# kalenforn/clip-based-cross-modal-hash

Hardware: AMD Instinct MI355X
Metric: Hamming query x gallery pairs/sec (fused mAP@all pass, DCMHT COCO-shaped 64-bit) (higher is better)
Workload: dtype u32; 1 GPU; configs[1] DCMHT COCO 64-bit retrieval: Q=5000 queries x R=117218 gallery items per GPU (x1 GPUs, contiguous shards), K=64 bits, C=80 classes, mAP@all; Q=5000, R_per_gpu=117218, K=64, C=80, parallelism=gallery-shard x1, query_blocks=1

## Files before the change

clip-based-cross-modal-hash_amd/csrc/xmh_scan.hip:

```cpp
#include "xmh_common.h"
#include <atomic>
#include <math.h>
#include <mutex>
#include <string.h>
#include <vector>
#include "xmh_scan_bits.h"
#include "xmh_scan_mfma.h"
#include "xmh_scan_kernels.h"

#include <stdlib.h>
#include <type_traits>

namespace {

constexpr int kSlotBudget64 = 9 * 1024;
constexpr int kSlotBudget32 = 5 * 1024;
constexpr int slots_for(int W, bool tern, int counter_bytes) {
    const int nbmax = (tern ? 64 : 32) * W + 1;
    const int budget = counter_bytes == 8 ? kSlotBudget64 : kSlotBudget32;
    const int cap = W > 8 ? 64 : 8;
    int S = 2;
    while (S < cap && nbmax * (64 / S) * counter_bytes > budget) S *= 2;
    return S;
}
inline int instance_words(int W) { return W <= 1 ? 1 : (W <= 2 ? 2 : (W <= 4 ? 4 : (W <= 8 ? 8 : (W <= 16 ? 16 : (W <= 32 ? 32 : 64))))); }
constexpr bool pair_cache_shape(int W, bool tern) { return !tern && (W == 1 || W == 2 || W == 4 || W == 8); }
// ... 247 lines not shown
    int W = 0, LW = 0;
    bool tern = false, cache = false;
    int S = 0, NW = 1;
    int nml = 0;
    int eb = 0; bool half = false;
    bool p32 = false, masked = false;
    unsigned gate = 0;
    bool stand_in = false;
};
struct ScanRoute {
    Launch p1;
    size_t cache_bytes = 0;
    int rank_bits = 0;
    Launch p2[3];
    int n2 = 0;
};

ScanRoute scan_route(const xmh_scan_plan& p, const ScanCall& c, Mode mode, const Overrides& ov, hipStream_t st) {
    ScanRoute r;
    const int K = c.K, C = c.C; const bool tern = c.tern; const int64_t R = c.R;
    const Family fam = pass1_family(K, tern, ov);
    const int W = ov.describe ? instance_words((K + 31) / 32) : (K + 31) / 32, LW = (C + 31) / 32;
    const bool lane_ok = ov.describe || (!ov.masked && lane_order_ok(st));
    r.cache_bytes = cache_for_workspace(p, K, tern, fam, c.ws_bytes);
    const bool cache = r.cache_bytes != 0;
    const bool mfma = fam != Family::kValu && LW <= 4 && lane_ok;
    Launch& h = r.p1;
    h.W = W; h.LW = LW; h.tern = tern; h.cache = cache; h.nml = LW <= 2 ? 1 : 2;
    if (!mfma) {
        h.cache = cache && pair_cache_shape(W, tern);
        h.S = h.cache ? cache_slots(W) : slots_for(W, tern, 4);
// ... 19 lines not shown
    const unsigned size_gate = sharded && (apc || apr2) ? kBySize : 0u;
    r.rank_bits = byte128 && apc ? 0 : rank_bits;
    auto add = [&](Kern kern, unsigned gate) -> Launch& { Launch& l = r.p2[r.n2++]; l.kern = kern; l.gate = gate; return l; };
    if (apc) {
        Launch& l = add(Kern::kApC, size_gate | (byte128 ? kByWrap : 0u));
        l.eb = 8; l.half = byte128; l.S = byte128 ? 8 : 4;
    }
    if (apr2) {
        Launch& l = add(Kern::kApR2, size_gate);
        l.W = W; l.LW = LW; l.nml = h.nml; l.NW = kAp2Waves; l.S = kAp2Groups;
    }
    if (apc16) {
        Launch& l = add(Kern::kApC, kByWidth);
        l.eb = 16; l.S = 8;
    }
    if ((apc || apr2) && !size_gate && !byte128) return r;
    Launch s;
    s.kern = Kern::kApS; s.W = tb ? 8 : W; s.LW = LW; s.tern = tern && !tb; s.masked = masked;
    s.cache = cache && !byte128 && !masked && pair_cache_shape(s.W, s.tern);
    s.stand_in = byte128 && apc;
    s.gate = size_gate | (s.stand_in ? kByWrap : 0u) | (r.rank_bits ? kByWidth : 0u);
    for (const bool p32 : {true, false}) {
        if (p32 ? r.rank_bits == 0 : apc16) continue;
        s.p32 = p32;
        s.S = s.cache ? cache_slots(s.W) : slots_for(s.W, s.tern, p32 ? 4 : 8);
        s.NW = s.S == 64 ? waves_for(s.W, s.tern) : 1;
        r.p2[r.n2++] = s;
    }
    return r;
}

// ... 80 lines not shown
    hipLaunchKernelGGL(kern, dim3(g.grid), dim3(g.block), g.lds, st, args...);
    return XMH_OK;
}

struct ScanCtx {
    const ScanCall& c;
    hipStream_t st;
    xmh_scan_plan p;
    ScanRoute r;
    WsLayout L;
    ScanArgs a;
    uint32_t kcap = 0xffffffffu;
    bool capped = false;
    template <typename T> T* at(size_t off) const { return reinterpret_cast<T*>(static_cast<char*>(c.ws) + off); }
    uint32_t* chunk_hist() const { return at<uint32_t>(L.chunk_hist); }
    const uint2* below() const { return at<uint2>(L.below); }
    uint2* tot() const { return at<uint2>(L.tot); }
    uint2* dpre() const { return at<uint2>(L.dpre); }
    uint32_t* cap_ws() const { return at<uint32_t>(L.cap); }
    float* ap_part() const { return at<float>(L.ap_part); }
    ScanArgs args(const Geom& g, bool cached) const { ScanArgs as = a; as.nqt = g.nqt; as.nrun = g.nrun; as.pair_cache = cached ? pair_cache() : nullptr; return as; }
    uint32_t* gate(int word = 0) const { return at<uint32_t>(L.gate) + word; }
    const uint32_t* gate_if(const Launch& l, unsigned g, int word) const { return (l.gate & g) ? gate(word) : nullptr; }
    uint4* pair_cache() const { return r.cache_bytes ? at<uint4>(L.pair_cache) : nullptr; }
};

int plan_call(const char* who, ScanCtx& x, const Overrides& ov) {
    if (const int rc = make_plan(x.c.Q, x.c.R, x.c.K, x.c.tern, &x.p, ov)) return rc;
    return check_common(who, x.c, x.p);
}
// ... 41 lines not shown
    hipLaunchKernelGGL(k_scan_touch, dim3(xmh::scan_grid_blocks(kTouchPerChunk, (int)p.nchunk)), dim3(256), 0, x.st, x.c.rbits, x.c.rlab, x.c.R, h.W, h.LW,
                       p.chunk, (int)p.nchunk, x.at<uint32_t>(x.L.tick), (int)((x.L.gate + 256 - x.L.tick) / 4));
    XMH_LAUNCH_CHECK("xmh_hamming_hist control words");
    const MfmaArgs a = r2_args(x.c, h, p, g.nqt);
    xmh::ProfScope prof("scan_hist", x.st);
    auto go = [&](auto kern, int NW, int NQ, bool cached, auto... wrap_word) { return start("xmh_hamming_hist", h, g, x.st, kern, NQ, NW, cached, a, chunk_hist, cache, wrap_word...); };
    if (h.kern == Kern::kHistR2w) {
        uint32_t* ovf = x.gate(kGateWrapped);
        return h.nml == 1 ? (h.cache ? go(k_scan_hist_r2w<1, 4, 2, true>, 4, 2, true, ovf) : go(k_scan_hist_r2w<1, 4, 2, false>, 4, 2, false, ovf))
                          : (h.cache ? go(k_scan_hist_r2w<2, 4, 2, true>, 4, 2, true, ovf) : go(k_scan_hist_r2w<2, 4, 2, false>, 4, 2, false, ovf));
    }
    return h.nml == 1 ? (h.cache ? go(k_scan_hist_r2<1, 4, 4, true>, 4, 4, true) : go(k_scan_hist_r2<1, 4, 4, false>, 4, 4, false))
                      : (h.cache ? go(k_scan_hist_r2<2, 4, 4, true>, 4, 4, true) : go(k_scan_hist_r2<2, 4, 4, false>, 4, 4, false));
}

int hamming_hist_impl(const ScanCall& c, uint32_t* hist_all, uint32_t* hist_rel, xmh_stream_t stream, const Overrides& ov) {
    ScanCtx x{c, xmh::as_stream(stream)};
    if (const int rc = plan_call("xmh_hamming_hist", x, ov)) return rc;
    route_call(x, Mode::kUnsharded, ov);
    const xmh_scan_plan& p = x.p;
    const Kern kern = x.r.p1.kern;
    if (kern == Kern::kHistS || kern == Kern::kHistB) XMH_HIP(hipMemsetAsync(x.at<char>(x.L.tick), 0, x.L.gate + 256 - x.L.tick, x.st));
    if (const int rc = kern == Kern::kHistS ? valu_hist(x) : mfma_hist(x)) return rc;
    XMH_LAUNCH_CHECK("xmh_hamming_hist");
    hipLaunchKernelGGL(k_scan_below, dim3((unsigned)p.nqtile, (unsigned)xmh::ceil_div(p.nbuckets, 4)), dim3(256), 0, x.st, x.chunk_hist(), (int)p.qpad,
                       (int)p.nbuckets, (int)p.nchunk, kern != Kern::kHistS ? kRelHi16 : 0u, x.at<uint2>(x.L.below), x.tot(), x.at<uint32_t>(x.L.tick), (int)c.Q, x.dpre(),
                       x.cap_ws(), x.gate(), hist_all, hist_rel);
    XMH_LAUNCH_CHECK("xmh_hamming_hist below");
    return XMH_OK;
}

}

extern "C" int xmh_scan_plan_make(int64_t Q, int64_t R, int K, int ternary, xmh_scan_plan* plan_host) {
    if (!plan_host) return xmh::fail(XMH_EINVAL, "xmh_scan_plan_make: null plan");
    return make_plan(Q, R, K, ternary, plan_host);
}

extern "C" size_t xmh_scan_pair_cache_bytes(int64_t Q, int64_t R, int K, int ternary) {
    xmh_scan_plan p;
    if (make_plan(Q, R, K, ternary, &p)) return 0;
    return pair_cache_bytes(p, K, ternary != 0, pass1_family(K, ternary != 0, {}));
}
// ... 19 lines not shown
    const ScanCall c{nullptr, nullptr, nullptr, nullptr, nullptr, nullptr, Q, R, K, C, nullptr, (size_t)p.ws_bytes, ternary != 0};
    const ScanRoute r = scan_route(p, c, Mode::kUnsharded, ov, nullptr);
    char p1[160], p2[200] = "", one[120];
    if (const int rc = describe_launch(r.p1, p1, sizeof(p1))) return rc;
    for (const bool p32 : {true, false})
        for (int i = 0; i < r.n2; ++i) {
            if (r.p2[i].stand_in || r.p2[i].p32 != p32) continue;
            if (const int rc = describe_launch(r.p2[i], one, sizeof(one))) return rc;
            const size_t at = strlen(p2);
            snprintf(p2 + at, sizeof(p2) - at, "%s%s", at ? "|" : "", one);
        }
    if ((size_t)snprintf(out, out_bytes, "pass1=%s;pass2=%s", p1, p2) >= out_bytes) return xmh::fail(XMH_EINVAL, "xmh_scan_describe: buffer too small");
    return XMH_OK;
}

extern "C" int xmh_hamming_hist(const uint32_t* qbits, const uint32_t* qzero, const uint32_t* qlab,
                                const uint32_t* rbits, const uint32_t* rzero, const uint32_t* rlab, int64_t Q, int64_t R,
                                int K, int C, void* ws, size_t ws_bytes, uint32_t* hist_all, uint32_t* hist_rel,
                                xmh_stream_t stream) {
    XMH_RANGE("xmh_hamming_hist (pass 1)");
    const ScanCall c{qbits, qzero, qlab, rbits, rzero, rlab, Q, R, K, C, ws, ws_bytes, qzero != nullptr};
    return hamming_hist_impl(c, hist_all, hist_rel, stream, {});
}

namespace {
int ap_offsets(const ScanCtx& x, const Pass2& o) {
    const xmh_scan_plan& p = x.p;
    if (o.mode == Mode::kUnsharded) return XMH_OK;
    if (o.mode == Mode::kAllToAll)
        hipLaunchKernelGGL(k_shard_scatter_offsets, dim3((unsigned)xmh::ceil_div(p.qpad, 256), (unsigned)p.nbuckets + 1), dim3(256), 0, x.st,
                           reinterpret_cast<const uint2*>(o.hist_g), (int)p.nbuckets, (int)(p.qpad / o.world), (int)x.c.Q, (int)p.qpad, o.k, x.dpre(), x.cap_ws(),
                           o.cap, x.gate(2));
    else if (o.mode == Mode::kTotals)
        hipLaunchKernelGGL(k_shard_offsets_dpre, dim3((unsigned)p.nqtile), dim3(256), 0, x.st, reinterpret_cast<const uint2*>(o.hist_g), o.world, o.rank,
                           (int)x.c.Q, (int)p.qpad, (int)p.nbuckets, o.k, x.dpre(), x.cap_ws(), o.cap, x.gate(2));
    else
        hipLaunchKernelGGL(k_scan_dpre, dim3((unsigned)p.nqtile), dim3(256), 0, x.st, (const uint2*)x.tot(), (int)x.c.Q, (int)p.qpad, (int)p.nbuckets, o.base_all,
                           o.base_rel, o.nrel_total, o.k, x.dpre(), x.cap_ws(), o.cap, (uint32_t*)nullptr, (uint32_t*)nullptr, (uint32_t*)nullptr, x.gate(2));
    XMH_LAUNCH_CHECK(o.mode == Mode::kAllToAll ? "xmh_hamming_map_sharded_offsets scatter" : (o.mode == Mode::kTotals ? "xmh_hamming_map_sharded offsets" : "xmh_hamming_ap dpre"));
    return XMH_OK;
}

int ap_launch_c(const ScanCtx& x, const Launch& l) {
    const Geom g = launch_geom(l, x.p, x.c.Q);
    const ScanArgs as = x.args(g, true);
    xmh::ProfScope prof("scan_ap", x.st);
    auto go = [&](auto kc, int S) {
        return start("xmh_hamming_ap", l, g, x.st, kc, S, 1, l.cache, as, x.below(), (const uint2*)x.dpre(), (const uint32_t*)x.cap_ws(), x.ap_part(),
                     x.gate_if(l, kBySize, 2), x.kcap, x.gate_if(l, kByWrap, kGateWrapped), x.gate_if(l, kByWidth, 0), l.gate & kByWidth ? x.r.rank_bits : 0);
    };
    if (l.eb == 16) return x.capped ? go(k_scan_ap_c<true, 16>, 8) : go(k_scan_ap_c<false, 16>, 8);
    if (l.half) return x.capped ? go(k_scan_ap_c<true, 8, true>, 8) : go(k_scan_ap_c<false, 8, true>, 8);
    return x.capped ? go(k_scan_ap_c<true, 8>, 4) : go(k_scan_ap_c<false, 8>, 4);
}

int ap_launch_r2(const ScanCtx& x, const Launch& l) {
    const Geom g = launch_geom(l, x.p, x.c.Q);
    const MfmaArgs ma = r2_args(x.c, l, x.p, g.nrun);
    xmh::ProfScope prof("scan_ap", x.st);
    auto go = [&](auto kern) {
        return start("xmh_hamming_ap", l, g, x.st, kern, kAp2Groups, kAp2Waves, l.cache, ma, x.below(), (const uint2*)x.dpre(), (const uint32_t*)x.cap_ws(), x.ap_part(),
                     x.gate_if(l, kBySize, 2), x.kcap);
    };
    return l.nml == 1 ? (x.capped ? go(k_scan_ap_r2<1, kAp2Waves, kAp2Groups, true>) : go(k_scan_ap_r2<1, kAp2Waves, kAp2Groups, false>))
// ... 91 lines not shown
    }
    if (nbad)
        return xmh::fail(XMH_EVERIFY_CODE, "xmh_scan_verify: %lld of %lld queries differ between the lane-order kernels and the masked re-derivation "
                         "(first: query %lld, AP sum %.9g vs %.9g, divisor %d vs %d)", (long long)nbad, (long long)Q, (long long)bad, a1[(size_t)bad], a0[(size_t)bad],
                         c1[(size_t)bad], c0[(size_t)bad]);
    return XMH_OK;
}

int hamming_ap_impl(const ScanCall& c, const Pass2& o, xmh_stream_t stream, const Overrides& ov) {
    ScanCtx x{c, xmh::as_stream(stream)};
    if (const int rc = plan_call("xmh_hamming_ap", x, ov)) return rc;
    if (!o.ap_sum || !o.cap) return xmh::fail(XMH_EINVAL, "xmh_hamming_ap: null output");
    const int ext = (o.base_all != nullptr) + (o.base_rel != nullptr) + (o.nrel_total != nullptr);
    if (ext != 0 && ext != 3) return xmh::fail(XMH_EINVAL, "xmh_hamming_ap: base_all, base_rel and nrel_total go together");
    route_call(x, o.mode, ov);
    x.kcap = o.k > 0 && o.k < (int64_t)0xffffffffll ? (uint32_t)o.k : 0xffffffffu;
    x.capped = o.k > 0;
    if (const int rc = ap_offsets(x, o)) return rc;
    for (int i = 0; i < x.r.n2; ++i) {
        const Launch& l = x.r.p2[i];
        if (const int rc = l.kern == Kern::kApC ? ap_launch_c(x, l) : (l.kern == Kern::kApR2 ? ap_launch_r2(x, l) : ap_launch_s(x, l))) return rc;
        XMH_LAUNCH_CHECK("xmh_hamming_ap");
    }
    if (const int rc = ap_reduce(x, o)) return rc;
    if (g_verify.load(std::memory_order_relaxed) && !ov.masked && o.mode == Mode::kUnsharded) return verify_against_masked(c, o, stream);
    return XMH_OK;
}

bool selfcheck_eval(const ScanCall& c, int force, std::vector<uint32_t>& hist, std::vector<double>& ap, std::vector<int32_t>& cap) {
    Overrides ov;
    ov.mfma = force;
    const int64_t Q = c.Q;
// ... 197 lines not shown
```

clip-based-cross-modal-hash_amd/csrc/xmh_scan_kernels.h:

```cpp
#pragma once
#include "xmh_scan_mfma.h"

namespace {
template <int W, int LW, bool TERN>
struct QueryRegs {
    uint32_t b[W];
    uint32_t z[TERN ? W : 1];
    uint32_t l[LW];
    __device__ __forceinline__ void load(const ScanArgs& a, int q) {
        const bool ok = q < a.Q;
#pragma unroll
        for (int w = 0; w < W; ++w) b[w] = ok ? a.qbits[(int64_t)q * W + w] : 0u;
        if (TERN) {
#pragma unroll
            for (int w = 0; w < W; ++w) z[w] = ok ? a.qzero[(int64_t)q * W + w] : 0xffffffffu;
        }
#pragma unroll
        for (int w = 0; w < LW; ++w) l[w] = ok ? a.qlab[(int64_t)q * LW + w] : 0u;
    }
};

template <int W, int LW, bool TERN>
struct Rec {
    uint32_t b[W];
// ... 12 lines not shown
        int live_n = 0, diff_n = 0;
#pragma unroll
        for (int w = 0; w < W; ++w) {
            const uint32_t live = ~(qr.z[w] | r.z[w]);
            live_n += __popc(live);
            diff_n += __popc((qr.b[w] ^ r.b[w]) & live);
        }
        d = K - live_n + 2 * diff_n;
    }
    uint32_t hit = qr.l[0] & r.l[0];
#pragma unroll
    for (int w = 1; w < LW; ++w) asm("v_and_or_b32 %0, %1, %2, %0" : "+v"(hit) : "v"(qr.l[w]), "v"(r.l[w]));
    asm("v_min_u32 %0, %1, 1" : "=v"(hit01) : "v"(hit));
}

constexpr uint32_t kRelHi16 = 0xffffffffu;
constexpr int kGateWrapped = 3;
__global__ __launch_bounds__(256) void k_scan_below(const uint32_t* __restrict__ chunk_hist, int qpad, int nb, int nchunk, uint32_t rel_scale,
                                                    uint2* __restrict__ below, uint2* __restrict__ tot, uint32_t* __restrict__ tickets, int Q,
                                                    uint2* __restrict__ dpre, uint32_t* __restrict__ nrel_ws, uint32_t* __restrict__ nrel_max,
                                                    uint32_t* __restrict__ hist_all, uint32_t* __restrict__ hist_rel) {
    __shared__ uint2 part[4][64];
    __shared__ int last;
    const int lane = threadIdx.x & 63, wq = threadIdx.x >> 6;
    const int d = blockIdx.y * 4 + wq;
    const int q = blockIdx.x * 64 + lane;
    const bool hi16 = rel_scale == kRelHi16;
    if (d < nb) {
        uint32_t ra = 0, rr = 0;
        int c = 0;
        for (; c + 4 <= nchunk; c += 4) {
            uint32_t h[4];
#pragma unroll
            for (int j = 0; j < 4; ++j) h[j] = chunk_hist[((int64_t)(c + j) * nb + d) * qpad + q];
#pragma unroll
            for (int j = 0; j < 4; ++j) {
                below[((int64_t)(c + j) * nb + d) * qpad + q] = make_uint2(ra, rr);
                const uint32_t rel = hi16 ? h[j] & 0xffffu : (rel_scale ? h[j] / rel_scale : h[j] >> 16);
                ra += hi16 ? h[j] >> 16 : (rel_scale ? h[j] - rel * rel_scale : h[j] & 0xffffu);
                rr += rel;
            }
        }
        for (; c < nchunk; ++c) {
// ... 878 lines not shown
```

clip-based-cross-modal-hash_amd/csrc/xmh_scan_mfma.h:

```cpp
#pragma once
#include "xmh_common.h"
#include "xmh_scan_map.h"
#include <type_traits>
#include <utility>

namespace {

constexpr int kMaxChunk = 32768;
constexpr uint32_t kF23 = 0x4B000000u;
constexpr int64_t kFloatBitsMaxItems = (1ll << 23) - 3;
constexpr int kMinChunk = 256;

struct ScanArgs {
    const uint32_t* qbits;
    const uint32_t* qzero;
    const uint32_t* qlab;
    const uint32_t* rbits;
    const uint32_t* rzero;
    const uint32_t* rlab;
    int Q, R, K;
    int chunk, nchunk, nqt, qpad, nb;
    uint4* pair_cache;
    int nrun;
};

__device__ __forceinline__ bool map_block(const ScanArgs& a, int& chunk_id, int& qtile) {
// ... 602 lines not shown
        uint32_t* __restrict__ out = chunk_hist + ((int64_t)chunk_id * a.nb) * a.qpad + (t16 + h) * 16;
        for (int e = lane; e < ncell; e += 64) out[(int64_t)(e >> 4) * a.qpad + (e & 15)] = lds[r2_cell(wave, h, e >> 4, e & 15)];
    }
    if (CACHE && dmax >= 65536u) *ovf = 1u;
}
#undef XMH_W_FUSED
#undef XMH_W_MFMA_F4
#undef XMH_W_MFMA
#undef XMH_W_MIN
#undef XMH_W_ADD

template <bool CAPPED, int EB, bool HALF = false>
__global__ __launch_bounds__(64) void k_scan_ap_c(ScanArgs a, const uint2* __restrict__ below, const uint2* __restrict__ dpre,
                                                  const uint32_t* __restrict__ cap_ws, float* __restrict__ ap_part,
                                                  const uint32_t* __restrict__ items_total, uint32_t kcap, const uint32_t* __restrict__ skip_if = nullptr,
                                                  const uint32_t* __restrict__ nrel_max = nullptr, int rank_bits = 0) {
    static_assert(!HALF || EB == 8, "the 8 x 8 geometry on one-byte entries");
    constexpr int QW = HALF ? 8 : 128 / EB, LOG_QW = QW == 16 ? 4 : 3, S = 64 / QW, EPW = HALF ? 2 : 32 / EB;
    extern __shared__ __attribute__((aligned(16))) uint32_t lds[];
    int chunk_id, qtile;
    if (!map_block(a, chunk_id, qtile)) return;
    if (items_total && (int64_t)*items_total > kFloatBitsMaxItems) return;
    if (skip_if && *skip_if != 0u) return;
    if (nrel_max && rank_bits > 0 && (uint64_t)(*nrel_max) + 2 < (1ull << (32 - rank_bits))) return;
    const int lane = threadIdx.x & 63;
    const int ql = lane & (QW - 1), slot = lane >> LOG_QW;
    const int q0 = qtile * QW, q = q0 + ql;
    const int ncell = a.nb * QW;
    unsigned long long* cnt = reinterpret_cast<unsigned long long*>(lds);
    {
        const uint2* __restrict__ pb = below + ((int64_t)chunk_id * a.nb) * a.qpad + q0;
        const uint2* __restrict__ pd = dpre + q0;
        auto pack = [](uint2 x, uint2 y) {
            return (unsigned long long)(kF23 + x.x + y.x + 1u) | ((unsigned long long)(kF23 + (0x7fffffu - (x.y + y.y + 1u))) << 32);
        };
        int e = lane;
        for (; e + 7 * 64 < ncell; e += 8 * 64) {
            uint2 x[8], y[8];
#pragma unroll
            for (int j = 0; j < 8; ++j) {
                const int ee = e + j * 64;
                const int64_t at = (int64_t)(ee >> LOG_QW) * a.qpad + (ee & (QW - 1));
                x[j] = pb[at];
                y[j] = pd[at];
            }
#pragma unroll
            for (int j = 0; j < 8; ++j) cnt[e + j * 64] = pack(x[j], y[j]);
        }
        for (; e < ncell; e += 64) {
            const int64_t at = (int64_t)(e >> LOG_QW) * a.qpad + (e & (QW - 1));
            cnt[e] = pack(pb[at], pd[at]);
        }
    }
    const uint32_t cntbase = (uint32_t)(uintptr_t)(__attribute__((address_space(3))) uint32_t*)lds + ql * 8;
    const float capf = CAPPED ? (float)min(cap_ws[q], kcap) : 0.0f;
    const int64_t lo = (int64_t)chunk_id * a.chunk;
    const int64_t hi = (lo + a.chunk < a.R) ? lo + a.chunk : a.R;
    float acc = 0.0f;
    auto credit = [&](unsigned long long old, uint32_t m) {
        const float rank = __uint_as_float((uint32_t)old) - 8388608.0f;
        const float ord = 16777215.0f - __uint_as_float((uint32_t)(old >> 32));
        if (CAPPED) m = ord <= capf ? m : 0u;
#ifdef XMH_ABL_AP_NORCP
        acc = fmaf(ord, __uint_as_float(__float_as_uint(rank) & m), acc);
#else
        acc = fmaf(ord, __uint_as_float(__float_as_uint(__builtin_amdgcn_rcpf(rank)) & m), acc);
#endif
    };
// ... 448 lines not shown
```

clip-based-cross-modal-hash_amd/xmh/_lib.py:

```python
from __future__ import annotations

import ctypes as C
import os

_HERE = os.path.dirname(os.path.abspath(__file__))
LIB_PATH = os.environ.get("XMH_LIB", os.path.join(_HERE, "libxmh.so"))

if not os.path.exists(LIB_PATH):
    raise ImportError(
        "libxmh.so not found at %s -- build it first (python -c 'import __graft_entry__ as g; g.build()' "
        "or make -C clip-based-cross-modal-hash_amd). There is no CPU fallback." % LIB_PATH)

import torch

lib = C.CDLL(LIB_PATH)

vp, i64, i32, sz = C.c_void_p, C.c_int64, C.c_int, C.c_size_t


class ScanPlan(C.Structure):
    _fields_ = [("chunk", i64), ("nchunk", i64), ("nqtile", i64), ("qpad", i64), ("nbuckets", i64), ("ws_bytes", sz)]


class Linear(C.Structure):
# ... 120 lines not shown
    "xmh_range_push": (i32, [C.c_char_p]),
    "xmh_range_pop": (i32, []),
    "xmh_scan_verify": (i32, [i32]),
    "xmh_prof_read": (i32, [C.c_char_p, C.POINTER(C.c_double), C.POINTER(i64)]),
    "xmh_pack_sign": (i32, [vp, i64, i32, vp, vp, vp, vp, vp]),
    "xmh_pack_pair_argmax": (i32, [vp, i64, i32, vp, vp, vp]),
    "xmh_unpack_pm1": (i32, [vp, vp, i64, i32, vp, vp]),
    "xmh_pack_labels": (i32, [vp, i32, i64, i32, vp, vp]),
    "xmh_hamming_dist": (i32, [vp, vp, vp, vp, i64, i64, i32, vp, vp, vp]),
    "xmh_label_sim": (i32, [vp, vp, i64, i64, i32, vp, vp]),
    "xmh_scan_plan_make": (i32, [i64, i64, i32, i32, C.POINTER(ScanPlan)]),
    "xmh_scan_pair_cache_bytes": (sz, [i64, i64, i32, i32]),
    "xmh_scan_pair_cache_offset": (sz, [i64, i64, i32, i32]),
    "xmh_scan_ws_bytes_nocache": (sz, [i64, i64, i32, i32]),
    "xmh_scan_describe": (i32, [i64, i64, i32, i32, i32, C.c_char_p, sz]),
    "xmh_hamming_hist": (i32, [vp, vp, vp, vp, vp, vp, i64, i64, i32, i32, vp, sz, vp, vp, vp]),
    "xmh_hamming_ap": (i32, [vp, vp, vp, vp, vp, vp, i64, i64, i32, i32, vp, sz, vp, vp, vp, i64, vp, vp, vp]),
    "xmh_hamming_map": (i32, [vp, vp, vp, vp, vp, vp, i64, i64, i32, i32, vp, sz, i64, vp, vp, vp, vp]),
    "xmh_scan_totals_offset": (sz, [i64, i64, i32, i32, C.POINTER(C.c_size_t)]),
    "xmh_hamming_map_sharded": (i32, [vp, vp, vp, vp, vp, vp, i64, i64, i32, i32, vp, sz, vp, i32, i32, i64, vp, vp, vp, vp]),
    "xmh_shard_slice_offsets": (i32, [vp, i32, i32, i32, vp, vp]),
    "xmh_hamming_map_sharded_offsets": (i32, [vp, vp, vp, vp, vp, vp, i64, i64, i32, i32, vp, sz, vp, i32, i64, vp, vp, vp, vp]),
    "xmh_calc_map_k_ws_bytes": (sz, [i64, i64, i32, i32]),
    "xmh_calc_map_k": (i32, [vp, vp, vp, vp, i64, i64, i32, i32, i64, vp, sz, C.POINTER(C.c_double), C.POINTER(i32), vp]),
    "xmh_map_finalize": (i32, [vp, vp, i64, vp, vp]),
    "xmh_shard_offsets": (i32, [vp, i32, i32, i64, i32, vp, vp, vp, vp]),
    "xmh_gemm_nt_f32": (i32, [vp, i64, vp, i64, vp, vp, i64, vp, i64, i64, i64, i64, i32, i32, vp]),
    "xmh_gemm_nt_h16": (i32, [vp, i64, vp, i64, vp, vp, i64, vp, i64, i64, i64, i64, i32, vp]),
    "xmh_gemm_nt_split16": (i32, [vp, i64, vp, vp, i64, vp, vp, i64, vp, i64, i64, i64, i64, i32, vp]),
    "xmh_cast_f32_to_f16": (i32, [vp, vp, i64, vp]),
    "xmh_layernorm_f32": (i32, [vp, i64, vp, vp, C.c_float, vp, i64, i64, i32, vp]),
# ... 176 lines not shown
```

clip-based-cross-modal-hash_amd/xmh/retrieval.py:

```python
from __future__ import annotations

import ctypes as C
import os
import warnings
from dataclasses import dataclass
from typing import Optional

import torch

from . import _lib
from ._lib import check, current_stream, lib, ptr

_DT = {torch.float32: 0, torch.int64: 1, torch.int32: 2, torch.uint8: 3, torch.bool: 3}


def _require_cuda(*tensors):
    for t in tensors:
        if t is None:
            continue
        if not t.is_cuda:
            raise RuntimeError("xmh ops need CUDA/HIP tensors (got a %s tensor); there is no CPU fallback" % t.device)
        if t.device.index != torch.cuda.current_device():
            raise RuntimeError("xmh op on a %s tensor while cuda:%d is current: wrap the call in torch.cuda.device(%d) "
                               "or torch.cuda.set_device first" % (t.device, torch.cuda.current_device(), t.device.index))
# ... 192 lines not shown
        if workspace is not None:
            self.plan, self.ws = workspace
            if self.ws.device != q.bits.device or self.ws.numel() < int(lib.xmh_scan_ws_bytes_nocache(q.n, r.n, q.K, 1 if self.qz is not None else 0)):
                raise ValueError("RankingScan: the workspace handed in does not fit this shape")
        else:
            self.plan, self.ws = _plan_and_workspace(q.n, r.n, q.K, self.qz is not None, q.bits.device)

    @property
    def workspace(self):
        return self.plan, self.ws

    def _common(self):
        return (ptr(self.q.bits), ptr(self.qz), ptr(self.qlab), ptr(self.r.bits), ptr(self.rz), ptr(self.rlab),
                self.q.n, self.r.n, self.q.K, self.C, ptr(self.ws), self.ws.numel())

    def histograms(self, want_totals: bool = True):
        ha = hr = None
        if want_totals:
            pair = torch.empty(2, self.q.n, self.plan.nbuckets, dtype=torch.int32, device=self.ws.device)
            ha, hr = pair[0], pair[1]
        check(lib.xmh_hamming_hist(*self._common(), ptr(ha), ptr(hr), current_stream()), "xmh_hamming_hist")
        return ha, hr

    def ap_sums(self, k: Optional[int] = None, base_all=None, base_rel=None, nrel_total=None):
        dev = self.ws.device
        ap = torch.empty(self.q.n, dtype=torch.float64, device=dev)
        cap = torch.empty(self.q.n, dtype=torch.int32, device=dev)
        kk = 0 if k is None else int(k)
        if k is not None and kk <= 0:
            raise ValueError("k must be positive or None")
        check(lib.xmh_hamming_ap(*self._common(), ptr(base_all), ptr(base_rel), ptr(nrel_total), kk, ptr(ap), ptr(cap),
                                 current_stream()), "xmh_hamming_ap")
        return ap, cap


    def map_all(self, k: Optional[int] = None):
# ... 173 lines not shown
```

clip-based-cross-modal-hash_amd/xmh/sharded.py:

```python
from __future__ import annotations

from typing import Optional, Sequence

import threading

import torch
import torch.distributed as dist


def shard_bounds(n: int, world: int) -> list:
    base, extra = divmod(n, world)
    out = [0]
    for r in range(world):
        out.append(out[-1] + base + (1 if r < extra else 0))
    return out


class HipShardOps:

    def __init__(self, q, qlab, r, rlab, C):
        from . import retrieval as R
        self._R = R
        self.q = R.widened(q)
        self.empty = r.n == 0
# ... 11 lines not shown
        return self._R.shard_offsets(hist_gathered, rank)

    def ap_sums(self, k, base_all, base_rel, nrel_total):
        if self.empty:
            cap = nrel_total if k is None else torch.clamp(nrel_total, max=int(k))
            return torch.zeros(self.q.n, dtype=torch.float64, device=nrel_total.device), cap.to(torch.int32)
        return self.scan.ap_sums(k, base_all, base_rel, nrel_total)

    def finalize(self, ap, cap):
        return self._R.map_finalize(ap, cap)

    def totals(self):
        if self.empty:
            p = self._R.scan_plan(self.q.n, 1, self.q.K, self._ternary)
            return torch.zeros(p.nbuckets, p.qpad, 2, dtype=torch.int32, device=self.q.bits.device)
        self.scan.histograms(False)
        return self.scan.totals()

    def map_partial(self, k, totals_gathered, rank):
        if self.empty:
            nrel = totals_gathered[:, :, : self.q.n, 1].sum(dim=(0, 1))
            cap = nrel if k is None else torch.clamp(nrel, max=int(k))
            z = torch.zeros(self.q.n, dtype=torch.float64, device=totals_gathered.device)
            return (z / cap.to(torch.float64)).sum().reshape(1) / self.q.n
        return self.scan.map_sharded(k, totals_gathered, rank)[0]


    def slice_offsets(self, totals_slices):
        return self._R.slice_offsets(totals_slices)

    def map_partial_offsets(self, k, offsets):
# ... 287 lines not shown
```

include/xmh.h:

```cpp
#ifndef XMH_H
#define XMH_H

#include <stddef.h>
#include <stdint.h>

#ifdef __cplusplus
extern "C" {
#endif

#define XMH_OK 0
#define XMH_EINVAL (-22)
#define XMH_ENOMEM (-12)
#define XMH_ENOTSUP (-95)
#define XMH_EHIP (-5)

#define XMH_DT_F32 0
#define XMH_DT_I64 1
#define XMH_DT_I32 2
#define XMH_DT_U8 3

typedef void* xmh_stream_t;

int xmh_version(void);
const char* xmh_build_id(void);
// ... 20 lines not shown

typedef struct xmh_scan_plan {
    int64_t chunk;
    int64_t nchunk;
    int64_t nqtile;
    int64_t qpad;
    int64_t nbuckets;
    size_t ws_bytes;
} xmh_scan_plan;

int xmh_scan_plan_make(int64_t Q, int64_t R, int K, int ternary, xmh_scan_plan* plan_host);
size_t xmh_scan_pair_cache_bytes(int64_t Q, int64_t R, int K, int ternary);
size_t xmh_scan_pair_cache_offset(int64_t Q, int64_t R, int K, int ternary);
size_t xmh_scan_ws_bytes_nocache(int64_t Q, int64_t R, int K, int ternary);
int xmh_scan_describe(int64_t Q, int64_t R, int K, int C, int ternary, char* out, size_t out_bytes);

int xmh_hamming_hist(const uint32_t* qbits, const uint32_t* qzero, const uint32_t* qlab,
                     const uint32_t* rbits, const uint32_t* rzero, const uint32_t* rlab,
                     int64_t Q, int64_t R, int K, int C, void* ws, size_t ws_bytes,
                     uint32_t* hist_all, uint32_t* hist_rel, xmh_stream_t stream);

int xmh_hamming_ap(const uint32_t* qbits, const uint32_t* qzero, const uint32_t* qlab,
                   const uint32_t* rbits, const uint32_t* rzero, const uint32_t* rlab,
                   int64_t Q, int64_t R, int K, int C, void* ws, size_t ws_bytes,
                   const uint32_t* base_all, const uint32_t* base_rel, const uint32_t* nrel_total,
                   int64_t k, double* ap_sum, int32_t* cap, xmh_stream_t stream);

int xmh_hamming_map(const uint32_t* qbits, const uint32_t* qzero, const uint32_t* qlab, const uint32_t* rbits,
                    const uint32_t* rzero, const uint32_t* rlab, int64_t Q, int64_t R, int K, int C, void* ws,
                    size_t ws_bytes, int64_t k, double* ap_sum, int32_t* cap, double* map_out, xmh_stream_t stream);
size_t xmh_calc_map_k_ws_bytes(int64_t Q, int64_t R, int K, int C);
int xmh_calc_map_k(const float* qB, const float* rB, const uint32_t* qlab, const uint32_t* rlab, int64_t Q, int64_t R, int K, int C,
                   int64_t k, void* ws, size_t ws_bytes, double* map_host, int32_t* flags_host, xmh_stream_t stream);
int xmh_map_finalize(const double* ap_sum, const int32_t* cap, int64_t Q, double* map_out, xmh_stream_t stream);
int xmh_shard_offsets(const uint32_t* hist_gathered, int world, int rank, int64_t Q, int nbuckets, uint32_t* base_all,
// ... 464 lines not shown
```

Baseline: 1782 billion pairs/s.

## Pack per-chunk below prefix counts into 16-bit pairs for unsharded AP pass

```diff
diff --git a/clip-based-cross-modal-hash_amd/csrc/xmh_scan.hip b/clip-based-cross-modal-hash_amd/csrc/xmh_scan.hip
--- a/clip-based-cross-modal-hash_amd/csrc/xmh_scan.hip
+++ b/clip-based-cross-modal-hash_amd/csrc/xmh_scan.hip
@@ -10,6 +10,7 @@
 
 #include <stdlib.h>
 #include <type_traits>
+#include <unordered_set>
 
 namespace {
 
@@ -287,7 +288,23 @@
     int rank_bits = 0;
     Launch p2[3];
     int n2 = 0;
+    bool tables32 = false;
 };
+
+std::mutex g_packed_mu;
+std::unordered_set<const void*> g_packed_ws;
+bool ws_packed(const void* ws) { std::lock_guard<std::mutex> lock(g_packed_mu); return g_packed_ws.count(ws) != 0; }
+void ws_set_packed(const void* ws, bool on) {
+    std::lock_guard<std::mutex> lock(g_packed_mu);
+    if (on) g_packed_ws.insert(ws); else g_packed_ws.erase(ws);
+}
+bool counts_fit16(int K, int64_t R) {
+    double peak = 1.0;
+    for (int i = 1; i <= K / 2; ++i) peak *= (double)(K - K / 2 + i) / (double)i;
+    peak = ldexp(peak, -K);
+    return 2.0 * peak * (double)R <= 65535.0;
+}
+bool tables_packed(bool apc_alone, Mode mode, int K, int64_t R) { return apc_alone && mode == Mode::kUnsharded && counts_fit16(K, R); }
 
 ScanRoute scan_route(const xmh_scan_plan& p, const ScanCall& c, Mode mode, const Overrides& ov, hipStream_t st) {
     ScanRoute r;
@@ -337,7 +354,10 @@
         Launch& l = add(Kern::kApC, kByWidth);
         l.eb = 16; l.S = 8;
     }
-    if ((apc || apr2) && !size_gate && !byte128) return r;
+    if ((apc || apr2) && !size_gate && !byte128) {
+        r.tables32 = tables_packed(apc, mode, K, R);
+        return r;
+    }
     Launch s;
     s.kern = Kern::kApS; s.W = tb ? 8 : W; s.LW = LW; s.tern = tern && !tb; s.masked = masked;
     s.cache = cache && !byte128 && !masked && pair_cache_shape(s.W, s.tern);
@@ -448,6 +468,7 @@
     bool capped = false;
     template <typename T> T* at(size_t off) const { return reinterpret_cast<T*>(static_cast<char*>(c.ws) + off); }
     uint32_t* chunk_hist() const { return at<uint32_t>(L.chunk_hist); }
+    uint32_t rel_scale() const { return r.p1.kern != Kern::kHistS ? kRelHi16 : 0u; }
     const uint2* below() const { return at<uint2>(L.below); }
     uint2* tot() const { return at<uint2>(L.tot); }
     uint2* dpre() const { return at<uint2>(L.dpre); }
@@ -519,19 +540,21 @@
                       : (h.cache ? go(k_scan_hist_r2<2, 4, 4, true>, 4, 4, true) : go(k_scan_hist_r2<2, 4, 4, false>, 4, 4, false));
 }
 
-int hamming_hist_impl(const ScanCall& c, uint32_t* hist_all, uint32_t* hist_rel, xmh_stream_t stream, const Overrides& ov) {
+int hamming_hist_impl(const ScanCall& c, uint32_t* hist_all, uint32_t* hist_rel, xmh_stream_t stream, const Overrides& ov, bool pass2_sharded = false) {
     ScanCtx x{c, xmh::as_stream(stream)};
     if (const int rc = plan_call("xmh_hamming_hist", x, ov)) return rc;
     route_call(x, Mode::kUnsharded, ov);
     const xmh_scan_plan& p = x.p;
     const Kern kern = x.r.p1.kern;
+    const bool packed = x.r.tables32 && !pass2_sharded;
     if (kern == Kern::kHistS || kern == Kern::kHistB) XMH_HIP(hipMemsetAsync(x.at<char>(x.L.tick), 0, x.L.gate + 256 - x.L.tick, x.st));
     if (const int rc = kern == Kern::kHistS ? valu_hist(x) : mfma_hist(x)) return rc;
     XMH_LAUNCH_CHECK("xmh_hamming_hist");
     hipLaunchKernelGGL(k_scan_below, dim3((unsigned)p.nqtile, (unsigned)xmh::ceil_div(p.nbuckets, 4)), dim3(256), 0, x.st, x.chunk_hist(), (int)p.qpad,
-                       (int)p.nbuckets, (int)p.nchunk, kern != Kern::kHistS ? kRelHi16 : 0u, x.at<uint2>(x.L.below), x.tot(), x.at<uint32_t>(x.L.tick), (int)c.Q, x.dpre(),
-                       x.cap_ws(), x.gate(), hist_all, hist_rel);
+                       (int)p.nbuckets, (int)p.nchunk, x.rel_scale(), x.at<uint2>(x.L.below), x.tot(), x.at<uint32_t>(x.L.tick), (int)c.Q, x.dpre(),
+                       x.cap_ws(), x.gate(), hist_all, hist_rel, packed, x.gate(kGateWide));
     XMH_LAUNCH_CHECK("xmh_hamming_hist below");
+    ws_set_packed(c.ws, packed);
     return XMH_OK;
 }
 
@@ -581,13 +604,39 @@
     return XMH_OK;
 }
 
+extern "C" size_t xmh_scan_gate_offset(int64_t Q, int64_t R, int K, int ternary) {
+    xmh_scan_plan p;
+    if (make_plan(Q, R, K, ternary, &p)) return (size_t)-1;
+    return ws_layout(p, 0).gate;
+}
+
+extern "C" int xmh_scan_tables_packed(int64_t Q, int64_t R, int K, int C, int ternary, int mode) {
+    if (mode < 0 || mode > 3) return xmh::fail(XMH_EINVAL, "xmh_scan_tables_packed: mode=%d", mode);
+    xmh_scan_plan p;
+    if (const int rc = make_plan(Q, R, K, ternary, &p)) return rc;
+    Overrides ov;
+    ov.describe = true;
+    const ScanCall c{nullptr, nullptr, nullptr, nullptr, nullptr, nullptr, Q, R, K, C, nullptr, (size_t)p.ws_bytes, ternary != 0};
+    static const Mode modes[4] = {Mode::kUnsharded, Mode::kBaseAll, Mode::kTotals, Mode::kAllToAll};
+    return scan_route(p, c, modes[mode], ov, nullptr).tables32 ? 1 : 0;
+}
+
 extern "C" int xmh_hamming_hist(const uint32_t* qbits, const uint32_t* qzero, const uint32_t* qlab,
                                 const uint32_t* rbits, const uint32_t* rzero, const uint32_t* rlab, int64_t Q, int64_t R,
                                 int K, int C, void* ws, size_t ws_bytes, uint32_t* hist_all, uint32_t* hist_rel,
                                 xmh_stream_t stream) {
     XMH_RANGE("xmh_hamming_hist (pass 1)");
     const ScanCall c{qbits, qzero, qlab, rbits, rzero, rlab, Q, R, K, C, ws, ws_bytes, qzero != nullptr};
-    return hamming_hist_impl(c, hist_all, hist_rel, stream, {});
+    return hamming_hist_impl(c, hist_all, hist_rel, stream, {}, hist_all != nullptr || hist_rel != nullptr);
+}
+
+extern "C" int xmh_hamming_hist_for(const uint32_t* qbits, const uint32_t* qzero, const uint32_t* qlab,
+                                    const uint32_t* rbits, const uint32_t* rzero, const uint32_t* rlab, int64_t Q, int64_t R,
+                                    int K, int C, void* ws, size_t ws_bytes, uint32_t* hist_all, uint32_t* hist_rel, int pass2_sharded,
+                                    xmh_stream_t stream) {
+    XMH_RANGE("xmh_hamming_hist (pass 1)");
+    const ScanCall c{qbits, qzero, qlab, rbits, rzero, rlab, Q, R, K, C, ws, ws_bytes, qzero != nullptr};
+    return hamming_hist_impl(c, hist_all, hist_rel, stream, {}, pass2_sharded != 0);
 }
 
 namespace {
@@ -611,10 +660,12 @@
 int ap_launch_c(const ScanCtx& x, const Launch& l) {
     const Geom g = launch_geom(l, x.p, x.c.Q);
     const ScanArgs as = x.args(g, true);
+    const uint32_t* wide = x.r.tables32 ? x.gate(kGateWide) : nullptr;
     xmh::ProfScope prof("scan_ap", x.st);
     auto go = [&](auto kc, int S) {
         return start("xmh_hamming_ap", l, g, x.st, kc, S, 1, l.cache, as, x.below(), (const uint2*)x.dpre(), (const uint32_t*)x.cap_ws(), x.ap_part(),
-                     x.gate_if(l, kBySize, 2), x.kcap, x.gate_if(l, kByWrap, kGateWrapped), x.gate_if(l, kByWidth, 0), l.gate & kByWidth ? x.r.rank_bits : 0);
+                     x.gate_if(l, kBySize, 2), x.kcap, x.gate_if(l, kByWrap, kGateWrapped), x.gate_if(l, kByWidth, 0), l.gate & kByWidth ? x.r.rank_bits : 0, wide,
+                     (const uint32_t*)x.chunk_hist(), x.rel_scale());
     };
     if (l.eb == 16) return x.capped ? go(k_scan_ap_c<true, 16>, 8) : go(k_scan_ap_c<false, 16>, 8);
     if (l.half) return x.capped ? go(k_scan_ap_c<true, 8, true>, 8) : go(k_scan_ap_c<false, 8, true>, 8);
@@ -736,8 +787,18 @@
     const int ext = (o.base_all != nullptr) + (o.base_rel != nullptr) + (o.nrel_total != nullptr);
     if (ext != 0 && ext != 3) return xmh::fail(XMH_EINVAL, "xmh_hamming_ap: base_all, base_rel and nrel_total go together");
     route_call(x, o.mode, ov);
+    const bool have_packed = ws_packed(c.ws);
+    if (x.r.tables32 && !have_packed) x.r.tables32 = false;
     x.kcap = o.k > 0 && o.k < (int64_t)0xffffffffll ? (uint32_t)o.k : 0xffffffffu;
     x.capped = o.k > 0;
+    if (!x.r.tables32 && have_packed) {
+        const xmh_scan_plan& p = x.p;
+        hipLaunchKernelGGL(k_scan_below, dim3((unsigned)p.nqtile, (unsigned)xmh::ceil_div(p.nbuckets, 4)), dim3(256), 0, x.st, x.chunk_hist(), (int)p.qpad,
+                           (int)p.nbuckets, (int)p.nchunk, x.rel_scale(), x.at<uint2>(x.L.below), x.tot(), (uint32_t*)nullptr, (int)x.c.Q, (uint2*)nullptr,
+                           (uint32_t*)nullptr, (uint32_t*)nullptr, (uint32_t*)nullptr, (uint32_t*)nullptr, false, (uint32_t*)nullptr);
+        XMH_LAUNCH_CHECK("xmh_hamming_ap below");
+        ws_set_packed(c.ws, false);
+    }
     if (const int rc = ap_offsets(x, o)) return rc;
     for (int i = 0; i < x.r.n2; ++i) {
         const Launch& l = x.r.p2[i];
diff --git a/clip-based-cross-modal-hash_amd/csrc/xmh_scan_kernels.h b/clip-based-cross-modal-hash_amd/csrc/xmh_scan_kernels.h
--- a/clip-based-cross-modal-hash_amd/csrc/xmh_scan_kernels.h
+++ b/clip-based-cross-modal-hash_amd/csrc/xmh_scan_kernels.h
@@ -50,19 +50,42 @@
     asm("v_min_u32 %0, %1, 1" : "=v"(hit01) : "v"(hit));
 }
 
-constexpr uint32_t kRelHi16 = 0xffffffffu;
 constexpr int kGateWrapped = 3;
+constexpr int kGateWide = 4;
 __global__ __launch_bounds__(256) void k_scan_below(const uint32_t* __restrict__ chunk_hist, int qpad, int nb, int nchunk, uint32_t rel_scale,
                                                     uint2* __restrict__ below, uint2* __restrict__ tot, uint32_t* __restrict__ tickets, int Q,
                                                     uint2* __restrict__ dpre, uint32_t* __restrict__ nrel_ws, uint32_t* __restrict__ nrel_max,
-                                                    uint32_t* __restrict__ hist_all, uint32_t* __restrict__ hist_rel) {
+                                                    uint32_t* __restrict__ hist_all, uint32_t* __restrict__ hist_rel, bool packed,
+                                                    uint32_t* __restrict__ wide) {
     __shared__ uint2 part[4][64];
     __shared__ int last;
     const int lane = threadIdx.x & 63, wq = threadIdx.x >> 6;
     const int d = blockIdx.y * 4 + wq;
     const int q = blockIdx.x * 64 + lane;
     const bool hi16 = rel_scale == kRelHi16;
-    if (d < nb) {
+    if (d < nb && packed) {
+        const int64_t cell = (int64_t)d * qpad + q, step = (int64_t)nb * qpad;
+        const uint32_t* __restrict__ src = chunk_hist + cell;
+        uint32_t* __restrict__ dst = reinterpret_cast<uint32_t*>(below) + cell;
+        uint32_t ra = 0, rr = 0;
+        for (int c0 = 0; c0 < nchunk; c0 += 16) {
+            uint32_t h[16];
+#pragma unroll
+            for (int j = 0; j < 16; ++j, src += step) h[j] = c0 + j < nchunk ? *src : 0u;
+#pragma unroll
+            for (int j = 0; j < 16; ++j, dst += step) {
+                if (c0 + j < nchunk) {
+                    *dst = (ra << 16) | rr;
+                    const uint2 n = chunk_counts(h[j], rel_scale);
+                    ra += n.x;
+                    rr += n.y;
+                }
+            }
+        }
+        if (ra > 0xffffu && q < Q) *wide = 1u;
+        __hip_atomic_store(reinterpret_cast<unsigned long long*>(tot + (int64_t)d * qpad + q), (unsigned long long)ra | ((unsigned long long)rr << 32),
+                           __ATOMIC_RELAXED, __HIP_MEMORY_SCOPE_AGENT);
+    } else if (d < nb) {
         uint32_t ra = 0, rr = 0;
         int c = 0;
         for (; c + 4 <= nchunk; c += 4) {
diff --git a/clip-based-cross-modal-hash_amd/csrc/xmh_scan_mfma.h b/clip-based-cross-modal-hash_amd/csrc/xmh_scan_mfma.h
--- a/clip-based-cross-modal-hash_amd/csrc/xmh_scan_mfma.h
+++ b/clip-based-cross-modal-hash_amd/csrc/xmh_scan_mfma.h
@@ -10,6 +10,12 @@
 constexpr uint32_t kF23 = 0x4B000000u;
 constexpr int64_t kFloatBitsMaxItems = (1ll << 23) - 3;
 constexpr int kMinChunk = 256;
+constexpr uint32_t kRelHi16 = 0xffffffffu;
+__device__ __forceinline__ uint2 chunk_counts(uint32_t h, uint32_t rel_scale) {
+    if (rel_scale == kRelHi16) return make_uint2(h >> 16, h & 0xffffu);
+    if (rel_scale == 0u) return make_uint2(h & 0xffffu, h >> 16);
+    return make_uint2(h % rel_scale, h / rel_scale);
+}
 
 struct ScanArgs {
     const uint32_t* qbits;
@@ -642,7 +648,8 @@
 __global__ __launch_bounds__(64) void k_scan_ap_c(ScanArgs a, const uint2* __restrict__ below, const uint2* __restrict__ dpre,
                                                   const uint32_t* __restrict__ cap_ws, float* __restrict__ ap_part,
                                                   const uint32_t* __restrict__ items_total, uint32_t kcap, const uint32_t* __restrict__ skip_if = nullptr,
-                                                  const uint32_t* __restrict__ nrel_max = nullptr, int rank_bits = 0) {
+                                                  const uint32_t* __restrict__ nrel_max = nullptr, int rank_bits = 0, const uint32_t* __restrict__ wide = nullptr,
+                                                  const uint32_t* __restrict__ chunk_hist = nullptr, uint32_t rel_scale = 0) {
     static_assert(!HALF || EB == 8, "the 8 x 8 geometry on one-byte entries");
     constexpr int QW = HALF ? 8 : 128 / EB, LOG_QW = QW == 16 ? 4 : 3, S = 64 / QW, EPW = HALF ? 2 : 32 / EB;
     extern __shared__ __attribute__((aligned(16))) uint32_t lds[];
@@ -663,23 +670,59 @@
             return (unsigned long long)(kF23 + x.x + y.x + 1u) | ((unsigned long long)(kF23 + (0x7fffffu - (x.y + y.y + 1u))) << 32);
         };
         int e = lane;
-        for (; e + 7 * 64 < ncell; e += 8 * 64) {
-            uint2 x[8], y[8];
-#pragma unroll
-            for (int j = 0; j < 8; ++j) {
-                const int ee = e + j * 64;
-                const int64_t at = (int64_t)(ee >> LOG_QW) * a.qpad + (ee & (QW - 1));
-                x[j] = pb[at];
-                y[j] = pd[at];
-            }
-#pragma unroll
-            for (int j = 0; j < 8; ++j) cnt[e + j * 64] = pack(x[j], y[j]);
-        }
-        for (; e < ncell; e += 64) {
-            const int64_t at = (int64_t)(e >> LOG_QW) * a.qpad + (e & (QW - 1));
-            cnt[e] = pack(pb[at], pd[at]);
-        }
-    }
+        if (wide == nullptr) {
+            for (; e + 7 * 64 < ncell; e += 8 * 64) {
+                uint2 x[8], y[8];
+#pragma unroll
+                for (int j = 0; j < 8; ++j) {
+                    const int ee = e + j * 64;
+                    const int64_t at = (int64_t)(ee >> LOG_QW) * a.qpad + (ee & (QW - 1));
+                    x[j] = pb[at];
+                    y[j] = pd[at];
+                }
+#pragma unroll
+                for (int j = 0; j < 8; ++j) cnt[e + j * 64] = pack(x[j], y[j]);
+            }
+            for (; e < ncell; e += 64) {
+                const int64_t at = (int64_t)(e >> LOG_QW) * a.qpad + (e & (QW - 1));
+                cnt[e] = pack(pb[at], pd[at]);
+            }
+        } else if (*wide == 0u) {
+            const uint32_t* __restrict__ pw = reinterpret_cast<const uint32_t*>(below) + ((int64_t)chunk_id * a.nb) * a.qpad + q0;
+            auto unpack = [](uint32_t w) { return make_uint2(w >> 16, w & 0xffffu); };
+            for (; e + 7 * 64 < ncell; e += 8 * 64) {
+                uint32_t w[8];
+                uint2 y[8];
+#pragma unroll
+                for (int j = 0; j < 8; ++j) {
+                    const int ee = e + j * 64;
+                    const int64_t at = (int64_t)(ee >> LOG_QW) * a.qpad + (ee & (QW - 1));
+                    w[j] = pw[at];
+                    y[j] = pd[at];
+                }
+#pragma unroll
+                for (int j = 0; j < 8; ++j) cnt[e + j * 64] = pack(unpack(w[j]), y[j]);
+            }
+            for (; e < ncell; e += 64) {
+                const int64_t at = (int64_t)(e >> LOG_QW) * a.qpad + (e & (QW - 1));
+                cnt[e] = pack(unpack(pw[at]), pd[at]);
+            }
+        } else {
+            const uint32_t* __restrict__ ph = chunk_hist + q0;
+            for (; e < ncell; e += 64) {
+                const int64_t at = (int64_t)(e >> LOG_QW) * a.qpad + (e & (QW - 1));
+                uint2 x = make_uint2(0u, 0u);
+#pragma unroll 4
+                for (int c = 0; c < chunk_id; ++c) {
+                    const uint2 n = chunk_counts(ph[((int64_t)c * a.nb) * a.qpad + at], rel_scale);
+                    x.x += n.x;
+                    x.y += n.y;
+                }
+                cnt[e] = pack(x, pd[at]);
+            }
+        }
+    }
+    asm volatile("" : "+s"(ap_part));
     const uint32_t cntbase = (uint32_t)(uintptr_t)(__attribute__((address_space(3))) uint32_t*)lds + ql * 8;
     const float capf = CAPPED ? (float)min(cap_ws[q], kcap) : 0.0f;
     const int64_t lo = (int64_t)chunk_id * a.chunk;
diff --git a/clip-based-cross-modal-hash_amd/xmh/_lib.py b/clip-based-cross-modal-hash_amd/xmh/_lib.py
--- a/clip-based-cross-modal-hash_amd/xmh/_lib.py
+++ b/clip-based-cross-modal-hash_amd/xmh/_lib.py
@@ -158,7 +158,10 @@
     "xmh_scan_pair_cache_offset": (sz, [i64, i64, i32, i32]),
     "xmh_scan_ws_bytes_nocache": (sz, [i64, i64, i32, i32]),
     "xmh_scan_describe": (i32, [i64, i64, i32, i32, i32, C.c_char_p, sz]),
+    "xmh_scan_tables_packed": (i32, [i64, i64, i32, i32, i32, i32]),
+    "xmh_scan_gate_offset": (sz, [i64, i64, i32, i32]),
     "xmh_hamming_hist": (i32, [vp, vp, vp, vp, vp, vp, i64, i64, i32, i32, vp, sz, vp, vp, vp]),
+    "xmh_hamming_hist_for": (i32, [vp, vp, vp, vp, vp, vp, i64, i64, i32, i32, vp, sz, vp, vp, i32, vp]),
     "xmh_hamming_ap": (i32, [vp, vp, vp, vp, vp, vp, i64, i64, i32, i32, vp, sz, vp, vp, vp, i64, vp, vp, vp]),
     "xmh_hamming_map": (i32, [vp, vp, vp, vp, vp, vp, i64, i64, i32, i32, vp, sz, i64, vp, vp, vp, vp]),
     "xmh_scan_totals_offset": (sz, [i64, i64, i32, i32, C.POINTER(C.c_size_t)]),
diff --git a/clip-based-cross-modal-hash_amd/xmh/retrieval.py b/clip-based-cross-modal-hash_amd/xmh/retrieval.py
--- a/clip-based-cross-modal-hash_amd/xmh/retrieval.py
+++ b/clip-based-cross-modal-hash_amd/xmh/retrieval.py
@@ -230,12 +230,13 @@
         return (ptr(self.q.bits), ptr(self.qz), ptr(self.qlab), ptr(self.r.bits), ptr(self.rz), ptr(self.rlab),
                 self.q.n, self.r.n, self.q.K, self.C, ptr(self.ws), self.ws.numel())
 
-    def histograms(self, want_totals: bool = True):
+    def histograms(self, want_totals: bool = True, sharded: Optional[bool] = None):
         ha = hr = None
         if want_totals:
             pair = torch.empty(2, self.q.n, self.plan.nbuckets, dtype=torch.int32, device=self.ws.device)
             ha, hr = pair[0], pair[1]
-        check(lib.xmh_hamming_hist(*self._common(), ptr(ha), ptr(hr), current_stream()), "xmh_hamming_hist")
+        sharded = want_totals if sharded is None else bool(sharded)
+        check(lib.xmh_hamming_hist_for(*self._common(), ptr(ha), ptr(hr), int(sharded), current_stream()), "xmh_hamming_hist")
         return ha, hr
 
     def ap_sums(self, k: Optional[int] = None, base_all=None, base_rel=None, nrel_total=None):
diff --git a/clip-based-cross-modal-hash_amd/xmh/sharded.py b/clip-based-cross-modal-hash_amd/xmh/sharded.py
--- a/clip-based-cross-modal-hash_amd/xmh/sharded.py
+++ b/clip-based-cross-modal-hash_amd/xmh/sharded.py
@@ -49,7 +49,7 @@
         if self.empty:
             p = self._R.scan_plan(self.q.n, 1, self.q.K, self._ternary)
             return torch.zeros(p.nbuckets, p.qpad, 2, dtype=torch.int32, device=self.q.bits.device)
-        self.scan.histograms(False)
+        self.scan.histograms(False, sharded=True)
         return self.scan.totals()
 
     def map_partial(self, k, totals_gathered, rank):
diff --git a/include/xmh.h b/include/xmh.h
--- a/include/xmh.h
+++ b/include/xmh.h
@@ -58,11 +58,17 @@
 size_t xmh_scan_pair_cache_offset(int64_t Q, int64_t R, int K, int ternary);
 size_t xmh_scan_ws_bytes_nocache(int64_t Q, int64_t R, int K, int ternary);
 int xmh_scan_describe(int64_t Q, int64_t R, int K, int C, int ternary, char* out, size_t out_bytes);
+int xmh_scan_tables_packed(int64_t Q, int64_t R, int K, int C, int ternary, int mode);
+size_t xmh_scan_gate_offset(int64_t Q, int64_t R, int K, int ternary);
 
 int xmh_hamming_hist(const uint32_t* qbits, const uint32_t* qzero, const uint32_t* qlab,
                      const uint32_t* rbits, const uint32_t* rzero, const uint32_t* rlab,
                      int64_t Q, int64_t R, int K, int C, void* ws, size_t ws_bytes,
                      uint32_t* hist_all, uint32_t* hist_rel, xmh_stream_t stream);
+int xmh_hamming_hist_for(const uint32_t* qbits, const uint32_t* qzero, const uint32_t* qlab,
+                         const uint32_t* rbits, const uint32_t* rzero, const uint32_t* rlab,
+                         int64_t Q, int64_t R, int K, int C, void* ws, size_t ws_bytes,
+                         uint32_t* hist_all, uint32_t* hist_rel, int pass2_sharded, xmh_stream_t stream);
 
 int xmh_hamming_ap(const uint32_t* qbits, const uint32_t* qzero, const uint32_t* qlab,
                    const uint32_t* rbits, const uint32_t* rzero, const uint32_t* rlab,
```

Result: faster. 1800 billion pairs/s (median of 6 runs) (+1.0%).
